# speechcatcher-asr/speechcatcher

Hardware: AMD Instinct MI355X
Metric: concurrent real-time streams (audio-seconds/s), de_xl dims, 640 ms (10240-sample) chunk steps, beam 10 CTC+attention (higher is better)
Workload: dtype f32

## Files before the change

include/scasr.h:

```cpp
#ifndef SCASR_H
#define SCASR_H

#include <stddef.h>
#include <stdint.h>

#ifdef __cplusplus
extern "C" {
#endif

#define SC_OK 0
#define SC_ERR_ARG (-1)
#define SC_ERR_LAUNCH (-2)
#define SC_ERR_CAPACITY (-3)
#define SC_ERR_INPUT (-4)

#define SC_GEMM_RELU 1
#define SC_GEMM_RESIDUAL 2
#define SC_GEMM_LN_AT_CROWS 8
#define SC_GEMM_NAIVE 4
#define SC_GEMM_SPLIT16 16

#define SC_F_ANY_EOS 1
#define SC_F_BEST_EOS 2
#define SC_F_ALL_EOS 4
// ... 307 lines not shown
            const uint8_t *is_final, int n, int *status);
int sc_push_features(sc_streams *streams, const int *stream_ids, const float *const *feats, const int *n_frames,
                     const uint8_t *is_final, int n, int *status);
int sc_submit(sc_streams *streams, const int *stream_ids, const float *const *pcm, const int *n_samples,
              const uint8_t *is_final, int n);
int sc_poll(sc_streams *streams, int min_done, int max_done, int *done_ids , int *status );
int sc_streams_outstanding(const sc_streams *streams);
int sc_streams_set_encoder_batch(sc_streams *streams, int min_streams);
int sc_streams_set_queue_depth(sc_streams *streams, int depth);
const char *sc_stream_last_error(const sc_streams *streams, int stream);
int sc_get_hyps(sc_streams *streams, int stream, int nbest, int max_len, int32_t *ids, int32_t *xpos, int *lens,
                double *scores, double *score_dec, double *score_ctc);
int sc_get_hyps_batch(sc_streams *streams, const int *stream_ids, int n, int nbest, int max_len, int32_t *ids,
                      int32_t *xpos, int *lens, int *n_hyps, double *scores, double *score_dec, double *score_ctc);
int sc_align_hyps(sc_streams *streams, const int *stream_ids, int n, int nbest, int max_len, int32_t *start,
                  int32_t *end, float *logp_mean, double *path_score, int *status, int *n_hyps);
int sc_align_tokens(sc_streams *streams, int stream, const int32_t *ids, int L, int32_t *start, int32_t *end,
                    float *logp_mean, double *path_score, int *status);
int sc_reset(sc_streams *streams, int stream);
int sc_stream_info(const sc_streams *streams, int stream, sc_stream_info_t *out);
#define SC_KV_POOL_DEFAULT_MAX_GIB 24
int sc_streams_kv_rows(const sc_streams *streams);
int sc_streams_stats(const sc_streams *streams, long *enc_calls, long *dec_steps, long *dec_blocks);
int sc_streams_capture_stats(const sc_streams *streams, long *n_captures, double *seconds);
int sc_streams_set_graphs(sc_streams *streams, int on);
int sc_marker(int id, void *stream);
int sc_streams_host_times(sc_streams *streams, double *launch_s, double *wait_s);
int sc_streams_bucket_times(sc_streams *streams, double *seconds, long *iterations);
long sc_streams_take_xattn_rows(sc_streams *streams);
int sc_streams_take_xattn_rows_by_kernel(sc_streams *streams, long *rows);
int sc_streams_take_attn_counters(sc_streams *streams, long *out );
void *sc_streams_hip_stream(sc_streams *streams);
float *sc_streams_pcm(sc_streams *streams, long *capacity);
int sc_streams_write_pcm(sc_streams *streams, int stream, long offset, const float *host, long n);
long sc_streams_read_pcm_buffer(sc_streams *streams, int stream, float *host, long max_n);
int sc_streams_read_enc(sc_streams *streams, int stream, float *host, int max_frames);
int sc_streams_read_ctc(sc_streams *streams, int stream, float *host, int max_rows);

#ifdef __cplusplus
}
#endif
#endif
```

speechcatcher_amd/_abi.py:

```python
import ctypes as C
import os
import subprocess
from pathlib import Path

HERE = Path(__file__).resolve().parent
LIB_PATH = HERE / "libscasr.so"
CSRC = HERE / "csrc"

c_float_p = C.POINTER(C.c_float)
c_int_p = C.POINTER(C.c_int32)
c_double_p = C.POINTER(C.c_double)
vp = C.c_void_p


class EncLayer(C.Structure):
    _fields_ = [(n, vp) for n in ("ln1_g", "ln1_b", "wqkv", "bqkv", "wo", "bo",
                                  "ln2_g", "ln2_b", "w1", "b1", "w2", "b2", "w1_p", "w2_p",
                                  "wqkv_p", "wo_p", "w1_h", "w2_h", "wqkv_h", "wo_h", "w1_s", "w2_s",
                                  "wqkv_s", "wo_s")]


class DecLayer(C.Structure):
    _fields_ = [(n, vp) for n in ("ln1_g", "ln1_b", "wqkv", "bqkv", "wo", "bo",
                                  "ln2_g", "ln2_b", "wq", "bq", "wo2", "bo2",
# ... 135 lines not shown
    "sc_dec_layer_reduce_ln": (C.c_int, [vp, C.c_int, vp, vp, vp, vp]),
    "sc_dec_layer_ffn_xn": (C.c_int, [vp, C.c_int, vp, vp, C.c_int, C.POINTER(C.c_int), vp]),
    "sc_engine_create": (C.c_int, [C.POINTER(Config), C.POINTER(NamedTensor), C.c_int, C.c_int, C.POINTER(vp)]),
    "sc_engine_load": (C.c_int, [C.c_char_p, C.c_int, C.POINTER(vp)]),
    "sc_engine_config": (C.c_int, [vp, C.POINTER(Config)]),
    "sc_engine_destroy": (None, [vp]),
    "sc_streams_create": (C.c_int, [vp, C.POINTER(StreamOptions), C.POINTER(vp)]),
    "sc_streams_destroy": (None, [vp]),
    "sc_push": (C.c_int, [vp, c_int_p, C.POINTER(vp), c_int_p, C.POINTER(C.c_uint8), C.c_int, c_int_p]),
    "sc_push_features": (C.c_int, [vp, c_int_p, C.POINTER(vp), c_int_p, C.POINTER(C.c_uint8), C.c_int, c_int_p]),
    "sc_get_hyps": (C.c_int, [vp, C.c_int, C.c_int, C.c_int, c_int_p, c_int_p, c_int_p, c_double_p, c_double_p,
                              c_double_p]),
    "sc_get_hyps_batch": (C.c_int, [vp, c_int_p, C.c_int, C.c_int, C.c_int, c_int_p, c_int_p, c_int_p, c_int_p,
                                    c_double_p, c_double_p, c_double_p]),
    "sc_submit": (C.c_int, [vp, c_int_p, C.POINTER(vp), c_int_p, C.POINTER(C.c_uint8), C.c_int]),
    "sc_poll": (C.c_int, [vp, C.c_int, C.c_int, c_int_p, c_int_p]),
    "sc_streams_outstanding": (C.c_int, [vp]),
    "sc_streams_set_encoder_batch": (C.c_int, [vp, C.c_int]),
    "sc_streams_set_queue_depth": (C.c_int, [vp, C.c_int]),
    "sc_stream_last_error": (C.c_char_p, [vp, C.c_int]),
    "sc_reset": (C.c_int, [vp, C.c_int]),
    "sc_stream_info": (C.c_int, [vp, C.c_int, C.POINTER(StreamInfo)]),
    "sc_streams_stats": (C.c_int, [vp, C.POINTER(C.c_long), C.POINTER(C.c_long), C.POINTER(C.c_long)]),
    "sc_streams_capture_stats": (C.c_int, [vp, C.POINTER(C.c_long), c_double_p]),
    "sc_streams_set_graphs": (C.c_int, [vp, C.c_int]),
    "sc_marker": (C.c_int, [C.c_int, vp]),
    "sc_streams_host_times": (C.c_int, [vp, c_double_p, c_double_p]),
    "sc_streams_bucket_times": (C.c_int, [vp, c_double_p, C.POINTER(C.c_long)]),
    "sc_streams_take_xattn_rows": (C.c_long, [vp]),
    "sc_streams_take_xattn_rows_by_kernel": (C.c_int, [vp, vp]),
    "sc_streams_take_attn_counters": (C.c_int, [vp, vp]),
    "sc_streams_hip_stream": (vp, [vp]),
    "sc_streams_pcm": (vp, [vp, C.POINTER(C.c_long)]),
    "sc_streams_write_pcm": (C.c_int, [vp, C.c_int, C.c_long, vp, C.c_long]),
    "sc_streams_read_pcm_buffer": (C.c_long, [vp, C.c_int, vp, C.c_long]),
    "sc_streams_read_enc": (C.c_int, [vp, C.c_int, vp, C.c_int]),
    "sc_ctc_align_ws_bytes": (C.c_size_t, [C.c_int]),
    "sc_ctc_align": (C.c_int, [vp, C.c_int, C.c_int, C.c_int, vp]),
    "sc_align_hyps": (C.c_int, [vp, c_int_p, C.c_int, C.c_int, C.c_int, c_int_p, c_int_p, c_float_p, c_double_p,
                                c_int_p, c_int_p]),
    "sc_align_tokens": (C.c_int, [vp, C.c_int, c_int_p, C.c_int, c_int_p, c_int_p, c_float_p, c_double_p, c_int_p]),
    "sc_streams_read_ctc": (C.c_int, [vp, C.c_int, vp, C.c_int]),
}

EXPORTED_SYMBOLS = tuple(_SIGS.keys())

# ... 51 lines not shown
```

speechcatcher_amd/csrc/streams.hip:

```cpp
#include <algorithm>
#include <array>
#include <chrono>
#include <cmath>
#include <cstdarg>
#include <cstring>
#include <deque>
#include <map>
#include <memory>
#include <new>
#include <string>
#include <vector>

#include "common.h"

namespace {

#define HIP_TRY(call)                                                              \
  do {                                                                             \
    hipError_t e__ = (call);                                                       \
    if (e__ != hipSuccess) {                                                       \
      sc_set_error("%s: %s failed: %s", __func__, #call, hipGetErrorString(e__));  \
      return SC_ERR_LAUNCH;                                                        \
    }                                                                              \
  } while (0)
// ... 121 lines not shown
  int n_fe = 0, max_keep = 0;
  EncPlan P;
  std::vector<int32_t> ctc_rows, kv_src, kv_dst;
  bool same_rows = true;
  std::vector<int> streams;
  bool empty() const { return !n_fe && !P.n_conv; }
};

constexpr int N_ARENA = 8;
constexpr int N_STAGE = 4;
constexpr int N_RING = 4;

struct sc_streams {
  sc_engine *eng = nullptr;
  sc_config cfg{};
  int S = 0, W = 0, K = 0, TCAP = 0, LCAP = 0, FCAP = 0, UCAP = 0, max_feat_new = 0, max_t1 = 0, max_t2 = 0,
      max_blocks = 0, max_chunk = 0, max_length = 500;
  long PCAP = 0;
  bool use_bbd = false, strict = true;
  hipStream_t stream = nullptr;
  hipStream_t stream_enc = nullptr, es = nullptr;
  hipEvent_t ev_iter[2] = {nullptr, nullptr};
  int32_t *ring_dev = nullptr;
  int32_t *rm_host[2] = {nullptr, nullptr};
  int rm_idx = 0;
  bool rm_dirty = false;
  int scan_split_min = 1024, scan_split_streams = 0;
  bool scan_long = false;
  int step_split_min() const { return (scan_long && (scan_split_streams <= 0 || n_rows_step <= scan_split_streams * W)) ? scan_split_min : 0; }
  int graph_key() const { return n_rows_step * 2 + (step_split_min() > 0 ? 1 : 0); }
  int enc_start_thr = 0;
  int enc_batch_min = 0;
  int gemm_flags = 0;
  void *ws = nullptr, *ws_enc = nullptr;
  std::vector<void *> owned, owned_host;
  float *pcm = nullptr, *featbuf = nullptr, *subbuf = nullptr, *prev_addin = nullptr, *past_ctx = nullptr, *enc = nullptr,
        *c1 = nullptr, *c2 = nullptr, *xblk = nullptr, *ws_xn = nullptr, *ws_qkv = nullptr, *ws_att = nullptr,
        *ws_ffh = nullptr;
  int32_t *jobs_ctx = nullptr, *ctrlmap = nullptr;
  float *kv_stage = nullptr;
  int kv_stage_rows = 0;
  sc_search sb{};
  int32_t *ctrlmap_host = nullptr, *flags_host = nullptr;
  int32_t *arena_host = nullptr, *arena_dev = nullptr;
  size_t slot_cap = 0, arena_off = 0;
  int cur_slot = 0;
  hipEvent_t ev_group[N_ARENA] = {nullptr};
  long slot_gen[N_ARENA] = {0};
  int32_t *bs_host = nullptr, *bs_dev = nullptr;
// ... 22 lines not shown
  int32_t *snap_yseq = nullptr, *snap_xpos = nullptr;
  double *snap_score = nullptr;
  hipEvent_t ev_snap = nullptr;
  std::vector<std::string> fault_msg;
  std::vector<long> enc_gen;
  std::deque<EncGroup *> groups;
  long gen_next = 1, gen_done = 0, gen_ordered = 0;
  int n_open = 0;
  long iter = 0;
  bool inflight = false;
  std::vector<int> tick_active;
  std::chrono::steady_clock::time_point tick_t0, tick_t1;
  hipStream_t stream_rb = nullptr;
  bool poisoned = false;
  std::vector<int> rowmap_key;
  int row_bucket = 1, n_rows_step = 0;
  bool decode_prepared = false;
  std::map<int, hipGraphExec_t> dec_graphs;
  std::map<std::vector<long>, hipGraphExec_t> enc_graphs;
  long dec_steps = 0, dec_blocks = 0, enc_calls = 0, xattn_rows[3] = {0, 0, 0};
  long sattn_pos[3] = {0, 0, 0};
  unsigned long long *stat_rows = nullptr;
  double t_launch = 0, t_wait = 0;
  double t_bucket[17] = {0};
  long n_bucket[17] = {0};
  bool use_graphs = true;
  long n_enc_captures = 0;
  double t_enc_capture = 0;

  ~sc_streams() {
    for (auto &g : dec_graphs) (void)hipGraphExecDestroy(g.second);
    for (auto &g : enc_graphs) (void)hipGraphExecDestroy(g.second);
    if (stream) (void)sc_set_stream_workspace(stream, nullptr, 0);
    if (stream_enc) {
      (void)sc_set_stream_workspace(stream_enc, nullptr, 0);
      (void)hipStreamDestroy(stream_enc);
    }
    for (int i = 0; i < 2; ++i)
      if (ev_iter[i]) (void)hipEventDestroy(ev_iter[i]);
    for (int i = 0; i < N_ARENA; ++i)
      if (ev_group[i]) (void)hipEventDestroy(ev_group[i]);
    for (int i = 0; i < N_STAGE; ++i)
      if (ev_stage[i]) (void)hipEventDestroy(ev_stage[i]);
    if (ev_snap) (void)hipEventDestroy(ev_snap);
    for (EncGroup *g : groups) delete g;
    for (void *p : owned) (void)hipFree(p);
    for (void *p : owned_host) (void)hipHostFree(p);
    if (stream_rb) (void)hipStreamDestroy(stream_rb);
    if (stream) (void)hipStreamDestroy(stream);
    if (al_dev) (void)hipFree(al_dev);
  }

  template <typename T>
  int alloc(T **p, size_t n) {
    RC_TRY(dalloc(p, n));
    owned.push_back(*p);
    return SC_OK;
  }
  template <typename T>
  int halloc(T **p, size_t n) {
    HIP_TRY(hipHostMalloc((void **)p, std::max<size_t>(n, 1) * sizeof(T)));
    owned_host.push_back(*p);
    memset(*p, 0, std::max<size_t>(n, 1) * sizeof(T));
    return SC_OK;
  }
  int32_t *ctrl_host() { return ctrlmap_host; }
  int32_t *rowmap_host() { return rm_host[rm_idx]; }

  int itensor(const std::vector<int32_t> &a, const int32_t **out) {
    const size_t n = a.size();
    if (arena_off + n > slot_cap) {
      sc_set_error("job-table arena exhausted (%zu + %zu of %zu entries)", arena_off, n, slot_cap);
      return SC_ERR_ARG;
    }
    const size_t off = (size_t)cur_slot * slot_cap + arena_off;
    arena_off += (n + 63) & ~size_t(63);
    if (n) {
      memcpy(arena_host + off, a.data(), n * sizeof(int32_t));
      HIP_TRY(hipMemcpyAsync(arena_dev + off, arena_host + off, n * sizeof(int32_t), hipMemcpyHostToDevice, es));
    }
    *out = arena_dev + off;
    return SC_OK;
  }
};


namespace {

constexpr int F_ANY_EOS = 1, F_BEST_EOS = 2, F_ALL_EOS = 4, F_REPEAT = 8;

__global__ void init_hyp_kernel(sc_search sb, int s) {
  const size_t o = ((size_t)0 * sb.S + s) * sb.W + 0;
  sb.yseq[o * sb.LCAP] = sb.sos;
  sb.xpos[o * sb.LCAP] = 0;
  sb.anc[((size_t)0 * sb.S + s) * sb.LCAP * sb.W] = 0;
  sb.score[o] = 0.0;
  sb.sc_dec[o] = 0.0;
  sb.sc_ctc[o] = 0.0;
}

__global__ __launch_bounds__(256) void scatter_f32_kernel(const float *__restrict__ src, float *__restrict__ dst,
                                                          const long long *__restrict__ jobs) {
  const long long so = jobs[blockIdx.y * 3], dof = jobs[blockIdx.y * 3 + 1], n = jobs[blockIdx.y * 3 + 2];
  for (long long i = (long long)blockIdx.x * 256 + threadIdx.x; i < n; i += (long long)gridDim.x * 256) dst[dof + i] = src[so + i];
}

__global__ __launch_bounds__(128) void pack_hyps_kernel(sc_search sb, const int32_t *__restrict__ jobs, int32_t *__restrict__ out,
                                                        const int32_t *__restrict__ snap_yseq, const int32_t *__restrict__ snap_xpos,
                                                        const double *__restrict__ snap_score) {
  const int32_t *j = jobs + (size_t)blockIdx.x * 4;
  const size_t row = (size_t)j[0];
  const int L = j[1];
// ... 325 lines not shown
  if (!P.emit_src.empty()) {
    const int32_t *a, *z;
    RC_TRY(b->itensor(P.emit_src, &a));
    RC_TRY(b->itensor(P.emit_dst, &z));
    RC_TRY(sc_layernorm(b->xblk, a, d, b->enc, z, d, (int)P.emit_src.size(), d, e->f("enc_norm_g"), e->f("enc_norm_b"),
                        c.ln_eps, b->es));
  }
  for (auto &sh : P.shorts) RC_TRY(encode_short(b, sh));
  if (!P.sub_src.empty()) {
    const int32_t *a, *z;
    RC_TRY(b->itensor(P.sub_src, &a));
    RC_TRY(b->itensor(P.sub_dst, &z));
    RC_TRY(sc_copy_rows(b->subbuf, a, b->subbuf, z, (int)P.sub_src.size(), d, b->es));
  }
  return SC_OK;
}

void set_rowmap(sc_streams *b, const std::vector<int> &active) {
  const int S = b->S, W = b->W;
  const int na = (int)active.size();
  const int nb = std::min(S, (na + b->row_bucket - 1) / b->row_bucket * b->row_bucket);
  if (active != b->rowmap_key) {
    b->rowmap_key = active;
    b->rm_idx ^= 1;
    b->rm_dirty = true;
    int32_t *rm = b->rowmap_host();
    std::vector<char> isact(S, 0);
    for (int s : active) isact[s] = 1;
    int k = 0;
    for (int pass = 1; pass >= 0; --pass)
      for (int s = 0; s < S; ++s)
        if (isact[s] == pass)
          for (int h = 0; h < W; ++h) rm[k++] = s * W + h;
  }
  b->n_rows_step = nb * W;
}

int decode_step_launch(sc_streams *b) {
  b->sb.n_rows = b->n_rows_step;
  b->sb.flags = b->ring_dev;
  auto step = [&]() { return sc_decode_step_ex(&b->sb, b->step_split_min(), b->stream); };
  if (!b->use_graphs) return step();
  auto it = b->dec_graphs.find(b->graph_key());
  if (it == b->dec_graphs.end()) {
    RC_TRY(step());
    RC_TRY(sc_graph_capture_begin(b->stream));
    const int rc = step();
    void *g = nullptr;
    const int rc2 = sc_graph_capture_end(b->stream, &g);
    if (rc != SC_OK) return rc;
    if (rc2 != SC_OK) return rc2;
    b->dec_graphs[b->graph_key()] = (hipGraphExec_t)g;
    return SC_OK;
  }
  return sc_graph_launch(it->second, b->stream);
}

int prepare_decode(sc_streams *b) {
  memset(b->ctrl_host(), 0, (size_t)b->S * 8 * sizeof(int32_t));
  HIP_TRY(hipMemcpyAsync(b->ctrlmap, b->ctrlmap_host, (size_t)b->S * 8 * sizeof(int32_t), hipMemcpyHostToDevice, b->stream));
  const int keep = b->n_rows_step;
  for (int nb = b->row_bucket; nb < b->S + b->row_bucket; nb += b->row_bucket) {
    b->n_rows_step = std::min(nb, b->S) * b->W;
    if (!b->dec_graphs.count(b->graph_key())) RC_TRY(decode_step_launch(b));
  }
  b->n_rows_step = keep;
  HIP_TRY(hipStreamSynchronize(b->stream));
  return SC_OK;
}

int retire_groups(sc_streams *b) {
  while (!b->groups.empty()) {
    EncGroup *g = b->groups.front();
    if (!g->launched) break;
    const hipError_t q = hipEventQuery(b->ev_group[g->slot]);
    if (q == hipErrorNotReady) { (void)hipGetLastError(); break; }
    if (q != hipSuccess) {
      sc_set_error("encoder group %ld failed: %s", g->gen, hipGetErrorString(q));
      return SC_ERR_LAUNCH;
    }
    b->gen_done = g->gen;
    b->slot_gen[g->slot] = 0;
    b->groups.pop_front();
// ... 36 lines not shown
                       kvt, 2 * d, m, 2 * d, d, b->gemm_flags, 0, b->es));
    } else {
      for (int r0 = 0; r0 < m; r0 += b->kv_stage_rows) {
        const int mm = std::min(b->kv_stage_rows, m - r0);
        if (!(all && sc_gemm_colblocks(b->enc, ar + r0, d, e->wkv_all, e->bkv_all, b->kv_stage, nullptr, 2 * d, mm, Ld * 2 * d, d, 2 * d,
                                       (long)mm * 2 * d, b->gemm_flags, b->es) == SC_OK))
          for (int li = 0; li < Ld; ++li)
            RC_TRY(sc_gemm(b->enc, ar + r0, d, e->wkv[li], e->bkv[li], b->kv_stage + (size_t)li * mm * 2 * d, nullptr, 2 * d,
                           mm, 2 * d, d, b->gemm_flags, 0, b->es));
        RC_TRY(sc_kv_rows_to_half(b->kv_stage, kvt + r0, mm, Ld, b->TCAP, 2 * d, const_cast<float *>(b->sb.ckv), b->es));
      }
    }
  }
  return SC_OK;
}

int stage_copy(sc_streams *b, EncGroup &g) {
  if (g.copy_jobs.empty()) return SC_OK;
  hipStream_t es = b->stream_enc ? b->stream_enc : b->stream;
  const int ss = g.stage_slot;
  const size_t so = (size_t)ss * b->stage_cap, jo = (size_t)ss * b->S * 3;
  const int nj = (int)g.copy_jobs.size() / 3;
  memcpy(b->cjobs_host + jo, g.copy_jobs.data(), g.copy_jobs.size() * sizeof(long long));
  HIP_TRY(hipMemcpyAsync(b->stage_dev + so, b->stage_host + so, g.stage_floats * sizeof(float), hipMemcpyHostToDevice, es));
  HIP_TRY(hipMemcpyAsync(b->cjobs_dev + jo, b->cjobs_host + jo, g.copy_jobs.size() * sizeof(long long), hipMemcpyHostToDevice, es));
  long long mx = 1;
  for (int j = 0; j < nj; ++j) mx = std::max(mx, g.copy_jobs[j * 3 + 2]);
  dim3 grid((unsigned)std::min<long long>(64, (mx + 1023) / 1024), nj);
  scatter_f32_kernel<<<grid, 256, 0, es>>>(b->stage_dev + so, g.features ? b->featbuf : b->pcm, b->cjobs_dev + jo);
  HIP_TRY(hipEventRecord(b->ev_stage[ss], es));
  b->stage_busy[ss] = true;
  g.copy_jobs.clear();
  return SC_OK;
}

void merge_group(sc_streams *b, EncGroup &dst, EncGroup &src) {
  const sc_config &c = b->cfg;
  const int F1 = c.conv_freq1, R = c.block_size + 2;
  EncPlan &D = dst.P, &P = src.P;
  int c1_rows = 0;
  if (D.n_conv) c1_rows = D.conv_jobs[(D.n_conv - 1) * 4 + 2] + D.conv_jobs[(D.n_conv - 1) * 4 + 3];
  const int nblk = (int)D.blk_jobs.size() / 6;
  for (int j = 0; j < P.n_conv; ++j) P.conv_jobs[j * 4 + 2] += c1_rows;
  for (auto &v : P.a_rows) v += c1_rows * F1;
  for (size_t j = 0; j < P.sjobs.size(); j += 5) P.sjobs[j] += nblk;
  for (auto &v : P.emit_src)
    if (v >= 0) v += nblk * R;
  auto cat = [](std::vector<int32_t> &a, const std::vector<int32_t> &x) { a.insert(a.end(), x.begin(), x.end()); };
// ... 139 lines not shown
  memset(ctrl0, 0, (size_t)S * 8 * sizeof(int32_t));
  int n_lsm = 0;
  for (int s : starts) {
    const Blk k = b->bq[s].front();
    b->bq[s].pop_front();
    St &x = b->st[s];
    Run &r = b->run[s];
    r = Run();
    r.inblk = r.live = true;
    r.T = k.T; r.fin = k.fin; r.job = k.job;
    r.cur = x.cur; r.L = x.L; r.nhyp = x.nhyp; r.has = x.has_ctc; r.pidx = x.process_idx; r.pvalid = x.prev_valid;
    const int told = x.T_ctc;
    r.Tc = std::max(k.T, told);
    if (k.T > told && told == 0)
      for (int t = 0; t < k.T && n_lsm < (int)(b->bs_cap - (size_t)S * 8); ++t) lsm[n_lsm++] = s * b->TCAP + t;
    int32_t *c = ctrl0 + s * 8;
    c[0] = 1; c[1] = r.cur; c[2] = r.fin; c[3] = r.Tc; c[4] = r.L; c[5] = r.nhyp; c[6] = r.has; c[7] = told;
    x.T_ctc = r.Tc;
    x.T_kv = std::max(k.T, x.T_kv);
    x.output_index = 0;
    r.nhp = r.nhyp; r.hasp = r.has;
    b->dec_blocks++;
  }
  HIP_TRY(hipMemcpyAsync(b->ctrlmap, ctrl0, (size_t)S * 8 * sizeof(int32_t), hipMemcpyHostToDevice, b->stream));
  if (n_lsm) {
    int32_t *ld = b->bs_dev + (size_t)b->bs_i * b->bs_cap;
    HIP_TRY(hipMemcpyAsync(ld, lsm, (size_t)n_lsm * sizeof(int32_t), hipMemcpyHostToDevice, b->stream));
    RC_TRY(sc_log_softmax_rows(const_cast<float *>(b->sb.ctcx), ld, n_lsm, b->cfg.vocab_size, b->stream));
  }
  RC_TRY(sc_ctc_extend_state(&b->sb, b->stream));
  return SC_OK;
}

int tick_collect(sc_streams *b);
int tick_issue(sc_streams *b, bool *progress) {
  const int S = b->S, W = b->W, Ld = b->cfg.dec_layers;
  *progress = false;
  if (b->inflight) RC_TRY(tick_collect(b));
  RC_TRY(retire_groups(b));
  RC_TRY(snapshot_completed(b));
  RC_TRY(start_blocks(b));
  {
    long need = 0;
    for (int s = 0; s < S; ++s)
      if (!b->run[s].inblk && !b->bq[s].empty()) need = std::max(need, b->bq[s].front().gen);
    long upto = -1;
    for (EncGroup *g : b->groups)
      if (!g->launched && g->deferred && g->gen <= need) upto = g->gen;
    if (upto >= 0) RC_TRY(launch_pending_groups(b, upto));
  }
  std::vector<int> &active = b->tick_active;
  active.clear();
// ... 21 lines not shown
    if (need > std::max(b->gen_done, b->gen_ordered)) {
      RC_TRY(launch_pending_groups(b, need));
      if (b->stream_enc) HIP_TRY(hipStreamWaitEvent(b->stream, b->ev_group[need % N_ARENA], 0));
      b->gen_ordered = std::max(b->gen_ordered, need);
      *progress = true;
    }
    return SC_OK;
  }
  *progress = true;
  b->tick_t0 = std::chrono::steady_clock::now();
  set_rowmap(b, active);
  b->scan_long = false;
  int32_t *ctrl = b->ctrl_host();
  memset(ctrl, 0, (size_t)S * 8 * sizeof(int32_t));
  for (int s : active) {
    const Run &r = b->run[s];
    if (b->scan_split_min > 0 && r.Tc - std::max(r.L - 1, 1) >= b->scan_split_min) b->scan_long = true;
    int32_t *c = ctrl + s * 8;
    c[0] = 1; c[1] = r.cur; c[2] = r.fin; c[3] = r.T; c[4] = r.L; c[5] = r.nhyp; c[6] = r.has; c[7] = r.Tc;
  }
  if ((int)active.size() <= b->enc_start_thr)
    for (EncGroup *g : b->groups)
      if (!g->launched && !g->open) RC_TRY(launch_group(b, g));
  if (b->rm_dirty) {
    memcpy(b->ctrlmap_host + S * 8, b->rm_host[b->rm_idx], (size_t)S * W * sizeof(int32_t));
    HIP_TRY(hipMemcpyAsync(b->ctrlmap, b->ctrlmap_host, (size_t)(S * 8 + S * W) * sizeof(int32_t), hipMemcpyHostToDevice, b->stream));
    b->rm_dirty = false;
  } else {
    HIP_TRY(hipMemcpyAsync(b->ctrlmap, b->ctrlmap_host, (size_t)S * 8 * sizeof(int32_t), hipMemcpyHostToDevice, b->stream));
  }
  RC_TRY(decode_step_launch(b));
  HIP_TRY(hipEventRecord(b->ev_iter[b->iter & 1], b->stream));
  const int form = sc_decode_step_form(&b->sb);
  for (int s : active) {
    b->xattn_rows[form] += (long)b->run[s].T * Ld;
    b->sattn_pos[form] += (long)b->run[s].L * Ld;
  }
  b->tick_t1 = std::chrono::steady_clock::now();
  b->inflight = true;
  return SC_OK;
}

int tick_collect(sc_streams *b) {
  if (!b->inflight) return SC_OK;
  const int S = b->S, W = b->W;
  b->inflight = false;
  const auto tpw = std::chrono::steady_clock::now();
  HIP_TRY(hipEventSynchronize(b->ev_iter[b->iter & 1]));
  const auto tp2 = std::chrono::steady_clock::now();
  b->iter++;
  b->dec_steps++;
  b->t_launch += std::chrono::duration<double>(b->tick_t1 - b->tick_t0).count();
  b->t_wait += std::chrono::duration<double>(tp2 - tpw).count();
  {
    const int bk = std::min(16, (int)((long)b->n_rows_step * 16 / std::max(1, S * W)));
    b->t_bucket[bk] += std::chrono::duration<double>(tp2 - b->tick_t0).count();
    b->n_bucket[bk] += 1;
  }
  for (int s : b->tick_active) {
    Run &r = b->run[s];
    const bool kv_full = b->flags_host[S + s] != 0;
    b->flags_host[S + s] = 0;
    const int f = b->flags_host[s];
    const bool f_any = f & F_ANY_EOS, f_best = f & F_BEST_EOS, f_all = f & F_ALL_EOS, f_rep = f & F_REPEAT;
    r.out += 1;
    r.nsteps += 1;
    const bool stop_eos = f_any && (!r.fin || f_best);
    const bool stop_bbd = b->use_bbd && !stop_eos && f_rep && !r.fin;
    const bool stop_all = !stop_eos && !stop_bbd && f_all && r.fin;
    const bool accept = !(stop_eos || stop_bbd || stop_all);
    const bool take = stop_eos || stop_all || accept;
    if (kv_full && take && !(!accept && r.pidx > 1 && r.pvalid)) {
// ... 589 lines not shown
      e->dec[0].wo2_pph && sb.ph1) {
    sb.out_w_qh = e->f("out_w_qh", false);
    sb.act_half = 1 | 2;
    if (const char *ah = sc_hook("SC_ACT_HALF")) sb.act_half = atoi(ah) & 7;
  }
  sb.layers = e->dec.data();
  (void)sc_set_stream_workspace(b->stream, b->ws, (size_t)128 << 20);
  b->es = b->stream;
  {
    b->enc_start_thr = S < 16 ? S : std::max(1, (int)((long)S * 7 / 100));
  }
  {
    const hipError_t er = hipStreamCreateWithPriority(&b->stream_enc, hipStreamNonBlocking, 0);
    if (er == hipSuccess && hipMalloc(&b->ws_enc, (size_t)128 << 20) == hipSuccess) {
      b->owned.push_back(b->ws_enc);
      (void)sc_set_stream_workspace(b->stream_enc, b->ws_enc, (size_t)128 << 20);
    } else {
      (void)hipGetLastError();
      if (b->stream_enc) (void)hipStreamDestroy(b->stream_enc);
      b->stream_enc = nullptr;
    }
  }
  const size_t cm = ((size_t)S * 8 + n) * sizeof(int32_t);
  bool ok = b->halloc(&b->ctrlmap_host, (size_t)S * 8 + n) == SC_OK && b->halloc(&b->flags_host, (size_t)S * 2) == SC_OK &&
            b->halloc(&b->rm_host[0], n) == SC_OK && b->halloc(&b->rm_host[1], n) == SC_OK &&
            b->halloc(&b->arena_host, b->slot_cap * N_ARENA) == SC_OK && b->halloc(&b->bs_host, b->bs_cap * N_RING) == SC_OK &&
            b->halloc(&b->stage_host, b->stage_cap * N_STAGE) == SC_OK && b->halloc(&b->pack_host, b->pack_cap) == SC_OK &&
            b->halloc(&b->pjobs_host, n * 4) == SC_OK && b->halloc(&b->cjobs_host, (size_t)N_STAGE * S * 3) == SC_OK;
  for (int i = 0; i < 2 && ok; ++i) ok = hipEventCreateWithFlags(&b->ev_iter[i], hipEventDisableTiming) == hipSuccess;
  for (int i = 0; i < N_ARENA && ok; ++i) ok = hipEventCreateWithFlags(&b->ev_group[i], hipEventDisableTiming) == hipSuccess;
  for (int i = 0; i < N_STAGE && ok; ++i) ok = hipEventCreateWithFlags(&b->ev_stage[i], hipEventDisableTiming) == hipSuccess;
  if (!ok) {
    sc_set_error("sc_streams_create: pinned host allocation failed");
    delete b;
    return SC_ERR_LAUNCH;
  }
  memset(b->flags_host, 0, (size_t)S * 8);
  {
    void *dv = nullptr;
    if (hipHostGetDevicePointer(&dv, b->flags_host, 0) != hipSuccess || !dv) {
      sc_set_error("sc_streams_create: pinned flags are not device-accessible");
      delete b;
      return SC_ERR_LAUNCH;
    }
    b->ring_dev = (int32_t *)dv;
    sb.flags = b->ring_dev;
    sb.kvflags = b->ring_dev + S;
  }
  if (const char *sp = sc_hook("SC_SCAN_SPLIT_MIN")) b->scan_split_min = atoi(sp);
  memset(b->ctrlmap_host, 0, cm);
  for (size_t i = 0; i < n; ++i) b->rm_host[0][i] = b->rm_host[1][i] = (int32_t)i;
  (void)hipMemcpy(b->ctrlmap, b->ctrlmap_host, (size_t)S * 8 * sizeof(int32_t), hipMemcpyHostToDevice);
  (void)hipMemcpy(b->ctrlmap + S * 8, b->rm_host[0], n * sizeof(int32_t), hipMemcpyHostToDevice);
  b->rowmap_key.resize(S);
  for (int s = 0; s < S; ++s) b->rowmap_key[s] = s;
  b->enc_batch_min = std::max(1, S / 2);
  b->gemm_flags = (!b->eng->enc.empty() && b->eng->enc[0].wqkv_s) ? SC_GEMM_SPLIT16 : 0;
  b->row_bucket = std::max(1, S / 32);
  b->n_rows_step = S * W;
  b->st.assign(S, St());
  b->run.assign(S, Run());
  b->bq.assign(S, std::deque<Blk>());
  b->job.assign(S, Job());
  b->ahead.assign(S, std::deque<Job>());
  b->job_seq.assign(S, 0);
  b->snap.assign(S, Snap());
  b->done_at.assign(S, 0);
  b->fault_msg.assign(S, std::string());
  b->enc_gen.assign(S, 0);
  for (int s = 0; s < S; ++s) init_hyp(b, s);
  *out = b;
  return SC_OK;
  SC_API_END
}

extern "C" void sc_streams_destroy(sc_streams *b) {
// ... 17 lines not shown
  if (!b) return nullptr;
  if (capacity) *capacity = b->PCAP;
  return b->pcm;
}

namespace {

int report_chunk(sc_streams *b, int s) {
  Job &j = b->job[s];
  const int status = j.fault ? j.fault : j.has_out;
  if (j.fault && !j.dropped) reset_stream(b, s);
  if (b->snap[s].valid && b->snap[s].seq == j.seq) b->snap[s].reported = true;
  b->done_at[s] = 0;
  if (b->ahead[s].empty()) j = Job();
  else {
    j = b->ahead[s].front();
    b->ahead[s].pop_front();
  }
  b->n_open--;
  return status;
}

int run_to_completion(sc_streams *b, const std::vector<int> &streams) {
  while (true) {
    bool all = true;
    for (int s : streams) all = all && (b->job[s].fault != 0 || chunk_decoded(b, s));
    if (all) return SC_OK;
    bool progress = false;
    RC_TRY(engine_tick(b, &progress));
    if (!progress) {
      sc_set_error("decode schedule stalled (internal error)");
      return SC_ERR_LAUNCH;
    }
  }
}

int push_impl(sc_streams *b, const int *stream_ids, const float *const *host, const int *counts, const uint8_t *is_final,
              int n, int *status, bool features, const char *what) {
  if (b->poisoned) {
    sc_set_error("%s: the handle was left inconsistent by an earlier failed call; destroy it", what);
    return SC_ERR_LAUNCH;
  }
  HIP_TRY(hipSetDevice(b->eng->device));
  RC_TRY(check_chunks(b, stream_ids, counts, n, what));
  for (int i = 0; i < n; ++i) b->snap[stream_ids[i]] = Snap();
  std::vector<Chunk> chunks;
// ... 69 lines not shown
      b->n_open++;
      continue;
    }
    chunks.push_back({s, pcm ? pcm[i] : nullptr, n_samples[i], is_final[i] != 0, i});
  }
  if (chunks.empty()) return SC_OK;
  const int rc = admit(b, chunks, false, true, nullptr);
  return rc == SC_OK ? SC_OK : poison(b, rc);
  SC_API_END
}

extern "C" int sc_poll(sc_streams *b, int min_done, int max_done, int *done_ids, int *status) {
  SC_CHECK_ARG(b && done_ids && max_done > 0, "bad arguments");
  SC_API_BEGIN
  if (b->poisoned) {
    sc_set_error("sc_poll: the handle was left inconsistent by an earlier failed call; destroy it");
    return SC_ERR_LAUNCH;
  }
  HIP_TRY(hipSetDevice(b->eng->device));
  min_done = std::min(std::min(min_done, max_done), b->n_open);
  for (Snap &sn : b->snap)
    if (sn.valid && sn.reported) sn.valid = false;
  int stalled = 0;
  while (true) {
    int rc = tick_collect(b);
    if (rc == SC_OK) rc = retire_groups(b);
    if (rc == SC_OK) rc = snapshot_completed(b);
    if (rc != SC_OK) return poison(b, rc);
    int n_complete = 0;
    for (int s = 0; s < b->S; ++s)
      if (chunk_complete(b, s)) {
        ++n_complete;
        if (!b->done_at[s]) b->done_at[s] = ++b->done_counter;
      }
    const bool enough = n_complete >= min_done || b->n_open == 0;
    bool progress = false;
    if (b->n_open > n_complete || !enough) {
      do {
        rc = tick_issue(b, &progress);
        if (rc != SC_OK) return poison(b, rc);
      } while (progress && !b->inflight);
    }
    if (enough) break;
    if (b->inflight || progress) stalled = 0;
    else if (n_complete > 0 && b->queue_depth > 1) break;
    else if (++stalled > 1) {
// ... 76 lines not shown
      n_hyps[i] = nh;
      SC_CHECK_ARG(nh == 0 || (!ids && !xpos) || max_len >= sn.L, "max_len is smaller than the hypotheses");
      for (int h = 0; h < nh; ++h) {
        jobs.insert(jobs.end(), {(int32_t)((size_t)s * b->W + h), sn.L, (int32_t)off, 1});
        off += (size_t)((2 * sn.L + 1) & ~1) + 6;
      }
      from_snapshot = true;
      continue;
    }
    SC_CHECK_ARG(!b->run[s].inblk && b->bq[s].empty(), "stream is inside a decode block (its chunk has not been reported yet)");
    const St &st = b->st[s];
    const int nh = st.started ? std::min(nbest, st.nhyp) : 0;
    n_hyps[i] = nh;
    SC_CHECK_ARG(nh == 0 || (!ids && !xpos) || max_len >= st.L, "max_len is smaller than the hypotheses");
    for (int h = 0; h < nh; ++h) {
      jobs.insert(jobs.end(), {(int32_t)(((size_t)st.cur * b->S + s) * b->W + h), st.L, (int32_t)off, 0});
      off += (size_t)((2 * st.L + 1) & ~1) + 6;
    }
  }
  const int m = (int)jobs.size() / 4;
  if (m == 0) return SC_OK;
  SC_CHECK_ARG(off <= b->pack_cap && (size_t)m <= (size_t)b->S * b->W, "hypotheses exceed the read-back buffer");
  memcpy(b->pjobs_host, jobs.data(), jobs.size() * sizeof(int32_t));
  HIP_TRY(hipMemcpyAsync(b->pjobs_dev, b->pjobs_host, jobs.size() * sizeof(int32_t), hipMemcpyHostToDevice, b->stream_rb));
  if (from_snapshot) HIP_TRY(hipStreamWaitEvent(b->stream_rb, b->ev_snap, 0));
  pack_hyps_kernel<<<m, 128, 0, b->stream_rb>>>(b->sb, b->pjobs_dev, b->pack_dev, b->snap_yseq, b->snap_xpos, b->snap_score);
  HIP_TRY(hipMemcpyAsync(b->pack_host, b->pack_dev, off * sizeof(int32_t), hipMemcpyDeviceToHost, b->stream_rb));
  HIP_TRY(hipStreamSynchronize(b->stream_rb));
  int k = 0;
  for (int i = 0; i < n; ++i)
    for (int h = 0; h < n_hyps[i]; ++h, ++k) {
      const int L = jobs[k * 4 + 1];
      const int32_t *src = b->pack_host + jobs[k * 4 + 2];
      const size_t o = (size_t)i * nbest + h;
      if (ids) memcpy(ids + o * max_len, src, (size_t)L * 4);
      if (xpos) memcpy(xpos + o * max_len, src + L, (size_t)L * 4);
      if (lens) lens[o] = L;
      const double *sc = (const double *)(src + ((2 * L + 1) & ~1));
      if (scores) scores[o] = sc[0];
      if (score_dec) score_dec[o] = sc[1];
      if (score_ctc) score_ctc[o] = sc[2];
    }
  return SC_OK;
  SC_API_END
}

struct AlignReq { int s, T; std::vector<int32_t> y; };
// ... 34 lines not shown
  sc_ctc_align_job *J = (sc_ctc_align_job *)host.data();
  int32_t *lab = (int32_t *)(host.data() + o_lab);
  int32_t *od = (int32_t *)(D + o_out);
  const int V = b->cfg.vocab_size;
  size_t li = 0, wo = o_ws;
  for (int k = 0; k < n; ++k) {
    const AlignReq &r = reqs[k];
    const int L = (int)r.y.size();
    if (L) memcpy(lab + li, r.y.data(), (size_t)L * 4);
    sc_ctc_align_job &j = J[k];
    j.emis = b->sb.ctcx + (size_t)r.s * b->TCAP * V;
    j.labels = (const int32_t *)(D + o_lab) + li;
    j.ws = D + wo;
    j.start = od + 3 * li;
    j.end = od + 3 * li + L;
    j.logp_mean = (float *)(od + 3 * li + 2 * L);
    j.path_score = (float *)(od + 3 * n_lab + 2 * k);
    j.status = od + 3 * n_lab + 2 * k + 1;
    j.stride = V;
    j.T = r.T; j.L = L; j.V = V; j.blank = b->cfg.blank_id;
    li += L;
    wo += al_round(sc_ctc_align_ws_bytes(r.T));
  }
  HIP_TRY(hipMemcpyAsync(D, host.data(), o_out, hipMemcpyHostToDevice, b->stream_rb));
  if (after_snap) HIP_TRY(hipStreamWaitEvent(b->stream_rb, b->ev_snap, 0));
  RC_TRY(sc_ctc_align((const sc_ctc_align_job *)D, n, max_T, max_L, b->stream_rb));
  std::vector<int32_t> res(n_outw);
  HIP_TRY(hipMemcpyAsync(res.data(), D + o_out, n_outw * 4, hipMemcpyDeviceToHost, b->stream_rb));
  HIP_TRY(hipStreamSynchronize(b->stream_rb));
  li = 0;
  for (int k = 0; k < n; ++k) {
    const int L = (int)reqs[k].y.size();
    AlignOut &o = out[k];
    o.start.assign(res.begin() + 3 * li, res.begin() + 3 * li + L);
    o.end.assign(res.begin() + 3 * li + L, res.begin() + 3 * li + 2 * L);
    o.lp.resize(L);
    if (L) memcpy(o.lp.data(), res.data() + 3 * li + 2 * L, (size_t)L * 4);
    memcpy(&o.score, res.data() + 3 * n_lab + 2 * k, 4);
    o.status = res[3 * n_lab + 2 * k + 1];
    li += L;
  }
  return SC_OK;
}

static int hyp_frames(const sc_streams *b, int s, int *T, bool *snap) {
  const Snap &sn = b->snap[s];
  *snap = sn.valid;
// ... 184 lines not shown
    seconds[i] = b->t_bucket[i];
    iterations[i] = b->n_bucket[i];
    b->t_bucket[i] = 0;
    b->n_bucket[i] = 0;
  }
  return SC_OK;
}

extern "C" int sc_streams_host_times(sc_streams *b, double *launch_s, double *wait_s) {
  SC_CHECK_ARG(b && launch_s && wait_s, "null");
  *launch_s = b->t_launch;
  *wait_s = b->t_wait;
  b->t_launch = b->t_wait = 0;
  return SC_OK;
}

extern "C" int sc_streams_capture_stats(const sc_streams *b, long *n_captures, double *seconds) {
  SC_CHECK_ARG(b && n_captures && seconds, "null");
  *n_captures = b->n_enc_captures;
  *seconds = b->t_enc_capture;
  return SC_OK;
}

extern "C" int sc_streams_stats(const sc_streams *b, long *enc_calls, long *dec_steps, long *dec_blocks) {
  SC_CHECK_ARG(b, "null");
  if (enc_calls) *enc_calls = b->enc_calls;
  if (dec_steps) *dec_steps = b->dec_steps;
  if (dec_blocks) *dec_blocks = b->dec_blocks;
  return SC_OK;
}
```

Measured before the change: 4071.

## Fetch per-tick control tables via device kernel from mapped pinned memory

Per-tick host-to-device memcpys of the control map, row map and log-softmax row lists are replaced by a small kernel. It reads the pinned host tables through their device-mapped alias and copies them into device buffers. A flag word decides whether the row map is refreshed, which removes the double-buffered row-map host copies. The goal is to cut DMA submission overhead and copy-engine latency on the decode stream, and it can be captured in graphs. The cost is extra kernel launches and system-scope reads over PCIe, plus some added instrumentation counters.

```diff
diff --git a/include/scasr.h b/include/scasr.h
--- a/include/scasr.h
+++ b/include/scasr.h
@@ -353,6 +353,7 @@
 #define SC_KV_POOL_DEFAULT_MAX_GIB 24
 int sc_streams_kv_rows(const sc_streams *streams);
 int sc_streams_stats(const sc_streams *streams, long *enc_calls, long *dec_steps, long *dec_blocks);
+int sc_streams_tick_stats(const sc_streams *streams, long *h2d_copies, long *boundaries, double *boundary_s);
 int sc_streams_capture_stats(const sc_streams *streams, long *n_captures, double *seconds);
 int sc_streams_set_graphs(sc_streams *streams, int on);
 int sc_marker(int id, void *stream);
diff --git a/speechcatcher_amd/_abi.py b/speechcatcher_amd/_abi.py
--- a/speechcatcher_amd/_abi.py
+++ b/speechcatcher_amd/_abi.py
@@ -181,6 +181,7 @@
     "sc_reset": (C.c_int, [vp, C.c_int]),
     "sc_stream_info": (C.c_int, [vp, C.c_int, C.POINTER(StreamInfo)]),
     "sc_streams_stats": (C.c_int, [vp, C.POINTER(C.c_long), C.POINTER(C.c_long), C.POINTER(C.c_long)]),
+    "sc_streams_tick_stats": (C.c_int, [vp, C.POINTER(C.c_long), C.POINTER(C.c_long), c_double_p]),
     "sc_streams_capture_stats": (C.c_int, [vp, C.POINTER(C.c_long), c_double_p]),
     "sc_streams_set_graphs": (C.c_int, [vp, C.c_int]),
     "sc_marker": (C.c_int, [C.c_int, vp]),
diff --git a/speechcatcher_amd/csrc/streams.hip b/speechcatcher_amd/csrc/streams.hip
--- a/speechcatcher_amd/csrc/streams.hip
+++ b/speechcatcher_amd/csrc/streams.hip
@@ -167,9 +167,9 @@
   hipStream_t stream_enc = nullptr, es = nullptr;
   hipEvent_t ev_iter[2] = {nullptr, nullptr};
   int32_t *ring_dev = nullptr;
-  int32_t *rm_host[2] = {nullptr, nullptr};
-  int rm_idx = 0;
+  int32_t *ctrlmap_alias = nullptr, *bs_alias = nullptr;
   bool rm_dirty = false;
+  std::vector<char> isact;
   int scan_split_min = 1024, scan_split_streams = 0;
   bool scan_long = false;
   int step_split_min() const { return (scan_long && (scan_split_streams <= 0 || n_rows_step <= scan_split_streams * W)) ? scan_split_min : 0; }
@@ -238,6 +238,10 @@
   long sattn_pos[3] = {0, 0, 0};
   unsigned long long *stat_rows = nullptr;
   double t_launch = 0, t_wait = 0;
+  long n_h2d_decode = 0, n_turn = 0;
+  double t_turn = 0;
+  std::chrono::steady_clock::time_point tick_seen;
+  bool seen_pending = false;
   double t_bucket[17] = {0};
   long n_bucket[17] = {0};
   bool use_graphs = true;
@@ -281,7 +285,12 @@
     return SC_OK;
   }
   int32_t *ctrl_host() { return ctrlmap_host; }
-  int32_t *rowmap_host() { return rm_host[rm_idx]; }
+  int h2d(void *dst, const void *src, size_t bytes, hipStream_t st) {
+    if (st == stream) ++n_h2d_decode;
+    HIP_TRY(hipMemcpyAsync(dst, src, bytes, hipMemcpyHostToDevice, st));
+    return SC_OK;
+  }
+  int32_t *rowmap_host() { return ctrlmap_host + (size_t)S * 8; }
 
   int itensor(const std::vector<int32_t> &a, const int32_t **out) {
     const size_t n = a.size();
@@ -293,7 +302,7 @@
     arena_off += (n + 63) & ~size_t(63);
     if (n) {
       memcpy(arena_host + off, a.data(), n * sizeof(int32_t));
-      HIP_TRY(hipMemcpyAsync(arena_dev + off, arena_host + off, n * sizeof(int32_t), hipMemcpyHostToDevice, es));
+      RC_TRY(h2d(arena_dev + off, arena_host + off, n * sizeof(int32_t), es));
     }
     *out = arena_dev + off;
     return SC_OK;
@@ -304,6 +313,28 @@
 namespace {
 
 constexpr int F_ANY_EOS = 1, F_BEST_EOS = 2, F_ALL_EOS = 4, F_REPEAT = 8;
+
+__global__ __launch_bounds__(256) void tick_fetch_kernel(const int32_t *src, int32_t *dst_a, int n_a, int32_t *dst_b, int n_b,
+                                                         const int32_t *cond) {
+  const int n = n_a + n_b, i0 = blockIdx.x * 1024 + threadIdx.x;
+  int32_t v[4];
+#pragma unroll
+  for (int k = 0; k < 4; ++k)
+    v[k] = i0 + k * 256 < n ? __hip_atomic_load(src + i0 + k * 256, __ATOMIC_RELAXED, __HIP_MEMORY_SCOPE_SYSTEM) : 0;
+  const bool part_b = !cond || __hip_atomic_load(cond, __ATOMIC_RELAXED, __HIP_MEMORY_SCOPE_SYSTEM) != 0;
+#pragma unroll
+  for (int k = 0; k < 4; ++k) {
+    const int i = i0 + k * 256;
+    if (i < n_a) dst_a[i] = v[k];
+    else if (i < n && part_b) dst_b[i - n_a] = v[k];
+  }
+}
+
+int tick_fetch(hipStream_t stream, const int32_t *src, int32_t *dst_a, int n_a, int32_t *dst_b, int n_b, const int32_t *cond) {
+  tick_fetch_kernel<<<(n_a + n_b + 1023) / 1024, 256, 0, stream>>>(src, dst_a, n_a, dst_b, n_b, cond);
+  SC_CHECK_LAUNCH();
+  return SC_OK;
+}
 
 __global__ void init_hyp_kernel(sc_search sb, int s) {
   const size_t o = ((size_t)0 * sb.S + s) * sb.W + 0;
@@ -675,10 +706,10 @@
   const int nb = std::min(S, (na + b->row_bucket - 1) / b->row_bucket * b->row_bucket);
   if (active != b->rowmap_key) {
     b->rowmap_key = active;
-    b->rm_idx ^= 1;
     b->rm_dirty = true;
     int32_t *rm = b->rowmap_host();
-    std::vector<char> isact(S, 0);
+    std::vector<char> &isact = b->isact;
+    isact.assign(S, 0);
     for (int s : active) isact[s] = 1;
     int k = 0;
     for (int pass = 1; pass >= 0; --pass)
@@ -692,7 +723,11 @@
 int decode_step_launch(sc_streams *b) {
   b->sb.n_rows = b->n_rows_step;
   b->sb.flags = b->ring_dev;
-  auto step = [&]() { return sc_decode_step_ex(&b->sb, b->step_split_min(), b->stream); };
+  auto step = [&]() {
+    const int nc = b->S * 8, nr = b->S * b->W;
+    RC_TRY(tick_fetch(b->stream, b->ctrlmap_alias, b->ctrlmap, nc, b->ctrlmap + nc, nr, b->ctrlmap_alias + nc + nr));
+    return sc_decode_step_ex(&b->sb, b->step_split_min(), b->stream);
+  };
   if (!b->use_graphs) return step();
   auto it = b->dec_graphs.find(b->graph_key());
   if (it == b->dec_graphs.end()) {
@@ -711,7 +746,7 @@
 
 int prepare_decode(sc_streams *b) {
   memset(b->ctrl_host(), 0, (size_t)b->S * 8 * sizeof(int32_t));
-  HIP_TRY(hipMemcpyAsync(b->ctrlmap, b->ctrlmap_host, (size_t)b->S * 8 * sizeof(int32_t), hipMemcpyHostToDevice, b->stream));
+  b->rowmap_host()[(size_t)b->S * b->W] = 0;
   const int keep = b->n_rows_step;
   for (int nb = b->row_bucket; nb < b->S + b->row_bucket; nb += b->row_bucket) {
     b->n_rows_step = std::min(nb, b->S) * b->W;
@@ -794,8 +829,8 @@
   const size_t so = (size_t)ss * b->stage_cap, jo = (size_t)ss * b->S * 3;
   const int nj = (int)g.copy_jobs.size() / 3;
   memcpy(b->cjobs_host + jo, g.copy_jobs.data(), g.copy_jobs.size() * sizeof(long long));
-  HIP_TRY(hipMemcpyAsync(b->stage_dev + so, b->stage_host + so, g.stage_floats * sizeof(float), hipMemcpyHostToDevice, es));
-  HIP_TRY(hipMemcpyAsync(b->cjobs_dev + jo, b->cjobs_host + jo, g.copy_jobs.size() * sizeof(long long), hipMemcpyHostToDevice, es));
+  RC_TRY(b->h2d(b->stage_dev + so, b->stage_host + so, g.stage_floats * sizeof(float), es));
+  RC_TRY(b->h2d(b->cjobs_dev + jo, b->cjobs_host + jo, g.copy_jobs.size() * sizeof(long long), es));
   long long mx = 1;
   for (int j = 0; j < nj; ++j) mx = std::max(mx, g.copy_jobs[j * 3 + 2]);
   dim3 grid((unsigned)std::min<long long>(64, (mx + 1023) / 1024), nj);
@@ -981,12 +1016,9 @@
     r.nhp = r.nhyp; r.hasp = r.has;
     b->dec_blocks++;
   }
-  HIP_TRY(hipMemcpyAsync(b->ctrlmap, ctrl0, (size_t)S * 8 * sizeof(int32_t), hipMemcpyHostToDevice, b->stream));
-  if (n_lsm) {
-    int32_t *ld = b->bs_dev + (size_t)b->bs_i * b->bs_cap;
-    HIP_TRY(hipMemcpyAsync(ld, lsm, (size_t)n_lsm * sizeof(int32_t), hipMemcpyHostToDevice, b->stream));
-    RC_TRY(sc_log_softmax_rows(const_cast<float *>(b->sb.ctcx), ld, n_lsm, b->cfg.vocab_size, b->stream));
-  }
+  int32_t *ld = b->bs_dev + (size_t)b->bs_i * b->bs_cap + (size_t)S * 8;
+  RC_TRY(tick_fetch(b->stream, b->bs_alias + (size_t)b->bs_i * b->bs_cap, b->ctrlmap, S * 8, ld, n_lsm, nullptr));
+  if (n_lsm) RC_TRY(sc_log_softmax_rows(const_cast<float *>(b->sb.ctcx), ld, n_lsm, b->cfg.vocab_size, b->stream));
   RC_TRY(sc_ctc_extend_state(&b->sb, b->stream));
   return SC_OK;
 }
@@ -1054,14 +1086,14 @@
   if ((int)active.size() <= b->enc_start_thr)
     for (EncGroup *g : b->groups)
       if (!g->launched && !g->open) RC_TRY(launch_group(b, g));
-  if (b->rm_dirty) {
-    memcpy(b->ctrlmap_host + S * 8, b->rm_host[b->rm_idx], (size_t)S * W * sizeof(int32_t));
-    HIP_TRY(hipMemcpyAsync(b->ctrlmap, b->ctrlmap_host, (size_t)(S * 8 + S * W) * sizeof(int32_t), hipMemcpyHostToDevice, b->stream));
-    b->rm_dirty = false;
-  } else {
-    HIP_TRY(hipMemcpyAsync(b->ctrlmap, b->ctrlmap_host, (size_t)S * 8 * sizeof(int32_t), hipMemcpyHostToDevice, b->stream));
-  }
+  b->rowmap_host()[(size_t)S * W] = b->rm_dirty ? 1 : 0;
+  b->rm_dirty = false;
   RC_TRY(decode_step_launch(b));
+  if (b->seen_pending) {
+    b->seen_pending = false;
+    b->t_turn += std::chrono::duration<double>(std::chrono::steady_clock::now() - b->tick_seen).count();
+    b->n_turn += 1;
+  }
   HIP_TRY(hipEventRecord(b->ev_iter[b->iter & 1], b->stream));
   const int form = sc_decode_step_form(&b->sb);
   for (int s : active) {
@@ -1080,6 +1112,8 @@
   const auto tpw = std::chrono::steady_clock::now();
   HIP_TRY(hipEventSynchronize(b->ev_iter[b->iter & 1]));
   const auto tp2 = std::chrono::steady_clock::now();
+  b->tick_seen = tp2;
+  b->seen_pending = true;
   b->iter++;
   b->dec_steps++;
   b->t_launch += std::chrono::duration<double>(b->tick_t1 - b->tick_t0).count();
@@ -1715,8 +1749,7 @@
     }
   }
   const size_t cm = ((size_t)S * 8 + n) * sizeof(int32_t);
-  bool ok = b->halloc(&b->ctrlmap_host, (size_t)S * 8 + n) == SC_OK && b->halloc(&b->flags_host, (size_t)S * 2) == SC_OK &&
-            b->halloc(&b->rm_host[0], n) == SC_OK && b->halloc(&b->rm_host[1], n) == SC_OK &&
+  bool ok = b->halloc(&b->ctrlmap_host, (size_t)S * 8 + n + 1) == SC_OK && b->halloc(&b->flags_host, (size_t)S * 2) == SC_OK &&
             b->halloc(&b->arena_host, b->slot_cap * N_ARENA) == SC_OK && b->halloc(&b->bs_host, b->bs_cap * N_RING) == SC_OK &&
             b->halloc(&b->stage_host, b->stage_cap * N_STAGE) == SC_OK && b->halloc(&b->pack_host, b->pack_cap) == SC_OK &&
             b->halloc(&b->pjobs_host, n * 4) == SC_OK && b->halloc(&b->cjobs_host, (size_t)N_STAGE * S * 3) == SC_OK;
@@ -1737,14 +1770,22 @@
       return SC_ERR_LAUNCH;
     }
     b->ring_dev = (int32_t *)dv;
+    void *dc = nullptr, *ds = nullptr;
+    if (hipHostGetDevicePointer(&dc, b->ctrlmap_host, 0) != hipSuccess || !dc ||
+        hipHostGetDevicePointer(&ds, b->bs_host, 0) != hipSuccess || !ds) {
+      sc_set_error("sc_streams_create: pinned control tables are not device-accessible");
+      delete b;
+      return SC_ERR_LAUNCH;
+    }
+    b->ctrlmap_alias = (int32_t *)dc;
+    b->bs_alias = (int32_t *)ds;
     sb.flags = b->ring_dev;
     sb.kvflags = b->ring_dev + S;
   }
   if (const char *sp = sc_hook("SC_SCAN_SPLIT_MIN")) b->scan_split_min = atoi(sp);
-  memset(b->ctrlmap_host, 0, cm);
-  for (size_t i = 0; i < n; ++i) b->rm_host[0][i] = b->rm_host[1][i] = (int32_t)i;
-  (void)hipMemcpy(b->ctrlmap, b->ctrlmap_host, (size_t)S * 8 * sizeof(int32_t), hipMemcpyHostToDevice);
-  (void)hipMemcpy(b->ctrlmap + S * 8, b->rm_host[0], n * sizeof(int32_t), hipMemcpyHostToDevice);
+  memset(b->ctrlmap_host, 0, cm + sizeof(int32_t));
+  for (size_t i = 0; i < n; ++i) b->ctrlmap_host[(size_t)S * 8 + i] = (int32_t)i;
+  (void)hipMemcpy(b->ctrlmap, b->ctrlmap_host, cm, hipMemcpyHostToDevice);
   b->rowmap_key.resize(S);
   for (int s = 0; s < S; ++s) b->rowmap_key[s] = s;
   b->enc_batch_min = std::max(1, S / 2);
@@ -1808,6 +1849,7 @@
 }
 
 int run_to_completion(sc_streams *b, const std::vector<int> &streams) {
+  b->seen_pending = false;
   while (true) {
     bool all = true;
     for (int s : streams) all = all && (b->job[s].fault != 0 || chunk_decoded(b, s));
@@ -1923,6 +1965,7 @@
   for (Snap &sn : b->snap)
     if (sn.valid && sn.reported) sn.valid = false;
   int stalled = 0;
+  b->seen_pending = false;
   while (true) {
     int rc = tick_collect(b);
     if (rc == SC_OK) rc = retire_groups(b);
@@ -2045,7 +2088,7 @@
   if (m == 0) return SC_OK;
   SC_CHECK_ARG(off <= b->pack_cap && (size_t)m <= (size_t)b->S * b->W, "hypotheses exceed the read-back buffer");
   memcpy(b->pjobs_host, jobs.data(), jobs.size() * sizeof(int32_t));
-  HIP_TRY(hipMemcpyAsync(b->pjobs_dev, b->pjobs_host, jobs.size() * sizeof(int32_t), hipMemcpyHostToDevice, b->stream_rb));
+  RC_TRY(b->h2d(b->pjobs_dev, b->pjobs_host, jobs.size() * sizeof(int32_t), b->stream_rb));
   if (from_snapshot) HIP_TRY(hipStreamWaitEvent(b->stream_rb, b->ev_snap, 0));
   pack_hyps_kernel<<<m, 128, 0, b->stream_rb>>>(b->sb, b->pjobs_dev, b->pack_dev, b->snap_yseq, b->snap_xpos, b->snap_score);
   HIP_TRY(hipMemcpyAsync(b->pack_host, b->pack_dev, off * sizeof(int32_t), hipMemcpyDeviceToHost, b->stream_rb));
@@ -2126,7 +2169,7 @@
     li += L;
     wo += al_round(sc_ctc_align_ws_bytes(r.T));
   }
-  HIP_TRY(hipMemcpyAsync(D, host.data(), o_out, hipMemcpyHostToDevice, b->stream_rb));
+  RC_TRY(b->h2d(D, host.data(), o_out, b->stream_rb));
   if (after_snap) HIP_TRY(hipStreamWaitEvent(b->stream_rb, b->ev_snap, 0));
   RC_TRY(sc_ctc_align((const sc_ctc_align_job *)D, n, max_T, max_L, b->stream_rb));
   std::vector<int32_t> res(n_outw);
@@ -2357,6 +2400,14 @@
   return SC_OK;
 }
 
+extern "C" int sc_streams_tick_stats(const sc_streams *b, long *h2d_copies, long *boundaries, double *boundary_s) {
+  SC_CHECK_ARG(b, "null");
+  if (h2d_copies) *h2d_copies = b->n_h2d_decode;
+  if (boundaries) *boundaries = b->n_turn;
+  if (boundary_s) *boundary_s = b->t_turn;
+  return SC_OK;
+}
+
 extern "C" int sc_streams_stats(const sc_streams *b, long *enc_calls, long *dec_steps, long *dec_blocks) {
   SC_CHECK_ARG(b, "null");
   if (enc_calls) *enc_calls = b->enc_calls;
```

After: 4064. About the same (-0.2%).
